# pl0q1n/RustyHGI

Hardware: AMD Instinct MI355X
Metric: Mpixels/s encode+decode, 4K grayscale level=4 Medium (higher is better)
Workload: dtype u8

## Files before the change

rustyhgi_amd/csrc/hgi_fused_impl.h:

```cpp
#include "hgi_dev.h"
#include "hgi_fastdiv.h"
#include "hgi_knobs.h"
#include "hgi_tilewalk.h"

namespace hgi {
namespace {

using namespace dev;

#ifndef HGI_TILE_H
#define HGI_TILE_H 64
#endif
#define HGI_LOG2(v) ((v) == 32 ? 5 : (v) == 16 ? 4 : (v) == 8 ? 3 : (v) == 4 ? 2 : 1)
#define HGI_CAT2(a, b) a##_##b
#define HGI_CAT(a, b) HGI_CAT2(a, b)
#define HGI_TILED(name) HGI_CAT(name, HGI_TILE_H)
#define HGI_LANE ((int)threadIdx.x)
constexpr int TW = kTileW;
constexpr int TH = HGI_TILE_H;
constexpr int MAXK = TH == 64 ? kFusedMaxLevels : TH == 32 ? kFusedMaxLevelsSmall : kFusedMaxLevelsTiny;
constexpr int NL = kThreads;
constexpr int CH = TW / 16;
constexpr int LCH = 3;
constexpr int HR = 6;
// ... 720 lines not shown
}

__device__ __forceinline__ void lattice_from_buf(const u8 *buf, u8 *rbuf, int nh)
{
    for (int i = HGI_LANE; i < (TH / 2 + nh) * CH; i += NL) {
        const int rr = i >> LCH, c = i & (CH - 1);
        *reinterpret_cast<v2u *>(rbuf + rr * S2 + 8 * c) = even_bytes(*reinterpret_cast<const v4u *>(buf + rr * S + 16 * c));
    }
    for (int i = HGI_LANE; i < HR * (TH / 2 + nh); i += NL) {
        const int hc = i / (TH / 2 + nh), rr = i - hc * (TH / 2 + nh);
        rbuf[RCOL + hc * HP2 + rr] = buf[HCOL + hc * HP + rr];
    }
}

__device__ __forceinline__ u32 gather_b0(v4u a)
{
    return __builtin_amdgcn_perm(a.y, a.x, 0x0c0c0400u) | __builtin_amdgcn_perm(a.w, a.z, 0x04000c0cu);
}

template <int INTERP, int EDGE = 0>
__device__ __forceinline__ void dec_level2_fast(u8 *buf, int rows = TH, int cols = TW)
{
    constexpr int N2 = (TH / 4) * CH;
#pragma unroll
    for (int it = 0; it < (N2 + NL - 1) / NL; ++it) {
        const bool on = N2 % NL == 0 || HGI_LANE + it * NL < N2;
        const int i = on ? HGI_LANE + it * NL : 0;
        u8 *r0 = buf + 2 * (i >> LCH) * S + 16 * (i & (CH - 1));
        v4u A = *reinterpret_cast<const v4u *>(r0);
        v4u B = *reinterpret_cast<const v4u *>(r0 + S);
        v4u C = *reinterpret_cast<const v4u *>(r0 + 2 * S);
        const int z0 = 2 * (i >> LCH);
        const bool last = (i & (CH - 1)) == CH - 1;
        u32 a16 = from_next_lane(A.x), c16 = from_next_lane(C.x);
        const u32 ha = buf[HCOL + z0], hc = buf[HCOL + z0 + 2];
        a16 = last ? ha : a16;
        c16 = last ? hc : c16;
        u32 ct = gather_b0(A), cb = gather_b0(C);
        u32 P = ct;
        if (INTERP == kInterpCrossed)
            P = pred4_crossed(ct, cb, __builtin_amdgcn_alignbyte(a16, ct, 1), __builtin_amdgcn_alignbyte(c16, cb, 1));
        u32 a0 = A.x, a1 = A.y, a2 = A.z, a3 = A.w, b0 = B.x, b1 = B.y, b2 = B.z, b3 = B.w;
        HGI_ADDB(a0, 2, P, 0); HGI_ADDB(a1, 2, P, 1); HGI_ADDB(a2, 2, P, 2); HGI_ADDB(a3, 2, P, 3);
        HGI_ADDB(b0, 0, P, 0); HGI_ADDB(b1, 0, P, 1); HGI_ADDB(b2, 0, P, 2); HGI_ADDB(b3, 0, P, 3);
        HGI_ADDB(b0, 2, P, 0); HGI_ADDB(b1, 2, P, 1); HGI_ADDB(b2, 2, P, 2); HGI_ADDB(b3, 2, P, 3);
        v4u An = {a0, a1, a2, a3}, Bn = {b0, b1, b2, b3};
        if (EDGE == 2 && cols < TW) {
            const v4u m = chunk_mask(cols - 16 * (i & (CH - 1)));
            An &= m;
            Bn &= m;
        }
        if (on && (!EDGE || 2 * z0 < rows)) *reinterpret_cast<v4u *>(r0) = An;
        if (on && (!EDGE || 2 * z0 + 2 < rows)) *reinterpret_cast<v4u *>(r0 + S) = Bn;
    }
}

template <int INTERP, int EDGE = 0>
__device__ __forceinline__ void dec_fine_fast(const u8 *buf, const Buf &b, const v4u (&odd)[NFINE], int rows = TH, int cols = TW)
{
    const int lane = HGI_LANE;
    const int rp0 = fine_pair0();
    const bool last = (lane & (CH - 1)) == CH - 1;
    const u8 *r0 = buf + rp0 * S + 16 * (lane & (CH - 1));
    const u8 *h0 = buf + HCOL + rp0;
    u32 voff = b.base + 2 * rp0 * b.W + 16 * (lane & (CH - 1));
#pragma unroll
    for (int it = 0; it < NFINE; ++it, r0 += (NL / CH) * S, h0 += NL / CH, voff += 2 * (NL / CH) * b.W) {
        v4u E = *reinterpret_cast<const v4u *>(r0);
        v4u O = odd[it];
        v4u F = *reinterpret_cast<const v4u *>(r0 + S);
        u32 e16 = from_next_lane(E.x), f16 = from_next_lane(F.x);
        const u32 he = h0[0], hf = h0[1];
        e16 = last ? he : e16;
        f16 = last ? hf : f16;
        uint2 c, fl;
        c.x = __builtin_amdgcn_perm(E.y, E.x, 0x06040200u);
        c.y = __builtin_amdgcn_perm(E.w, E.z, 0x06040200u);
        fl.x = __builtin_amdgcn_perm(F.y, F.x, 0x06040200u);
        fl.y = __builtin_amdgcn_perm(F.w, F.z, 0x06040200u);
        u32 P0, P1;
        pred8<INTERP>(c, e16, fl, f16, P0, P1);
        u32 e0 = E.x, e1 = E.y, e2 = E.z, e3 = E.w, o0 = O.x, o1 = O.y, o2 = O.z, o3 = O.w;
        HGI_ADDB(e0, 1, P0, 0); HGI_ADDB(e0, 3, P0, 1); HGI_ADDB(e1, 1, P0, 2); HGI_ADDB(e1, 3, P0, 3);
        HGI_ADDB(e2, 1, P1, 0); HGI_ADDB(e2, 3, P1, 1); HGI_ADDB(e3, 1, P1, 2); HGI_ADDB(e3, 3, P1, 3);
        HGI_ADDB(o0, 0, P0, 0); HGI_ADDB(o0, 1, P0, 0); HGI_ADDB(o0, 2, P0, 1); HGI_ADDB(o0, 3, P0, 1);
        HGI_ADDB(o1, 0, P0, 2); HGI_ADDB(o1, 1, P0, 2); HGI_ADDB(o1, 2, P0, 3); HGI_ADDB(o1, 3, P0, 3);
        HGI_ADDB(o2, 0, P1, 0); HGI_ADDB(o2, 1, P1, 0); HGI_ADDB(o2, 2, P1, 1); HGI_ADDB(o2, 3, P1, 1);
        HGI_ADDB(o3, 0, P1, 2); HGI_ADDB(o3, 1, P1, 2); HGI_ADDB(o3, 2, P1, 3); HGI_ADDB(o3, 3, P1, 3);
        v4u r0v = {e0, e1, e2, e3}, r1v = {o0, o1, o2, o3};
        if (EDGE == 2) {
            const int y = 2 * (rp0 + it * (NL / CH));
            store_rows_edge(r0v, r1v, b.rd, voff, __builtin_amdgcn_readfirstlane(b.W), cols - 16 * (lane & (CH - 1)), y < rows, y + 1 < rows);
        } else {
            store_row_pair(r0v, r1v, b.rd, voff, __builtin_amdgcn_readfirstlane(b.W));
        }
    }
}

template <int INTERP, bool IDENT, int EDGE = 0>
__device__ __forceinline__ void enc_level2_fast(u8 *buf, u8 *rbuf, const u8 *slut, Tile tl, u32 W, u32 H)
{
    const int rows = EDGE ? (int)(H - tl.Y0) : TH, cols = EDGE ? (int)(W - tl.X0) : TW;
    constexpr int N2 = (TH / 4) * CH, NIT = (N2 + NL - 1) / NL;
#pragma unroll
    for (int it = 0; it < NIT; ++it) {
        const bool on = N2 % NL == 0 || HGI_LANE + it * NL < N2;
        const int i = on ? HGI_LANE + it * NL : 0;
        const int g = i >> LCH, c = i & (CH - 1);
        u8 *r0 = buf + 2 * g * S + 16 * c;
        u8 *q0 = rbuf + 2 * g * S2 + 8 * c;
        const v4u A = *reinterpret_cast<const v4u *>(r0);
        const v4u B = *reinterpret_cast<const v4u *>(r0 + S);
        const v2u cu = *reinterpret_cast<const v2u *>(q0);
        const v2u cl = *reinterpret_cast<const v2u *>(q0 + 2 * S2);
        const u32 hu = rbuf[RCOL + 2 * g], hl = rbuf[RCOL + 2 * g + 2];
        LDS_ORDER();
        const bool last = c == CH - 1;
        u32 c8 = from_next_lane(cu.x), l8 = from_next_lane(cl.x);
        c8 = last ? hu : c8;
        l8 = last ? hl : l8;
        u32 ct = __builtin_amdgcn_perm(cu.y, cu.x, 0x06040200u), cb = __builtin_amdgcn_perm(cl.y, cl.x, 0x06040200u);
        u32 P = ct;
        if (INTERP == kInterpCrossed)
            P = pred4_crossed(ct, cb, __builtin_amdgcn_alignbyte(c8, ct, 1), __builtin_amdgcn_alignbyte(l8, cb, 1));
        u32 a0 = A.x, a1 = A.y, a2 = A.z, a3 = A.w, b0 = B.x, b1 = B.y, b2 = B.z, b3 = B.w;
        v2u n0, n1;
        if (IDENT) {
            const u32 pA = __builtin_amdgcn_perm(P, P, 0x0c010c00u), pB = __builtin_amdgcn_perm(P, P, 0x0c030c02u);
            n0.x = __builtin_amdgcn_perm(a0, ct, 0x0c010c00u) | __builtin_amdgcn_perm(a1, a0, 0x060c020cu);
            n0.y = __builtin_amdgcn_perm(a0, ct, 0x0c030c02u) | __builtin_amdgcn_perm(a3, a2, 0x060c020cu);
            n1.x = __builtin_amdgcn_perm(b1, b0, 0x06040200u);
            n1.y = __builtin_amdgcn_perm(b3, b2, 0x06040200u);
            const u32 m2 = 0x00FF0000u, m02 = 0x00FF00FFu;
            a0 = (a0 & ~m2) | (sub4(a0, pA << 16) & m2);
            a1 = (a1 & ~m2) | (sub4(a1, pA & m2) & m2);
            a2 = (a2 & ~m2) | (sub4(a2, pB << 16) & m2);
            a3 = (a3 & ~m2) | (sub4(a3, pB & m2) & m2);
            const u32 p0 = (pA & 0xFFu) * 0x00010001u, p1 = ((pA >> 16) & 0xFFu) * 0x00010001u;
            const u32 p2 = (pB & 0xFFu) * 0x00010001u, p3 = ((pB >> 16) & 0xFFu) * 0x00010001u;
            b0 = (b0 & ~m02) | (sub4(b0, p0) & m02);
            b1 = (b1 & ~m02) | (sub4(b1, p1) & m02);
            b2 = (b2 & ~m02) | (sub4(b2, p2) & m02);
            b3 = (b3 & ~m02) | (sub4(b3, p3) & m02);
        } else {
            const u32 NP = ~P;
            Q_PIX4(slut, P, NP, a0, 2, 0, a1, 2, 1, a2, 2, 2, a3, 2, 3);
            Q_PIX4(slut, P, NP, b0, 0, 0, b1, 0, 1, b2, 0, 2, b3, 0, 3);
            Q_PIX4(slut, P, NP, b0, 2, 0, b1, 2, 1, b2, 2, 2, b3, 2, 3);
            n0.x = __builtin_amdgcn_perm(ct, ct, 0x0c010c00u);
            n0.y = __builtin_amdgcn_perm(ct, ct, 0x0c030c02u);
            n1.x = 0;
            n1.y = 0;
            Q_REC(n0.x, 1, a0, 2, P, 0); Q_REC(n0.x, 3, a1, 2, P, 1); Q_REC(n0.y, 1, a2, 2, P, 2); Q_REC(n0.y, 3, a3, 2, P, 3);
            Q_REC(n1.x, 0, b0, 0, P, 0); Q_REC(n1.x, 1, b0, 2, P, 0); Q_REC(n1.x, 2, b1, 0, P, 1); Q_REC(n1.x, 3, b1, 2, P, 1);
            Q_REC(n1.y, 0, b2, 0, P, 2); Q_REC(n1.y, 1, b2, 2, P, 2); Q_REC(n1.y, 2, b3, 0, P, 3); Q_REC(n1.y, 3, b3, 2, P, 3);
        }
        v4u An = {a0, a1, a2, a3}, Bn = {b0, b1, b2, b3};
        if (EDGE == 2 && cols < TW) {
            const v4u m = chunk_mask(cols - 16 * c);
            const v2u m2 = chunk_mask2(cols - 16 * c);
            An &= m;
            Bn &= m;
            n0 &= m2;
            n1 &= m2;
        }
        if (on && (!EDGE || 4 * g < rows)) {
            *reinterpret_cast<v4u *>(r0) = An;
            *reinterpret_cast<v2u *>(q0) = n0;
        }
        if (on && (!EDGE || 4 * g + 2 < rows)) {
            *reinterpret_cast<v4u *>(r0 + S) = Bn;
            *reinterpret_cast<v2u *>(q0 + S2) = n1;
        }
        __builtin_amdgcn_sched_barrier(0);
    }
    LDS_ORDER();
    HGI_MARK("halo");
    enc_halo_pass<INTERP, IDENT>(buf, rbuf, slut, 2, tl, W, H);
}

template <int INTERP, bool IDENT, int EDGE = 0>
__device__ __forceinline__ void enc_fine_fast(const u8 *buf, const u8 *rbuf, const u8 *slut, const Buf &b,
                                              const v4u (&odd)[NFINE], int rows = TH, int cols = TW)
{
    const int lane = HGI_LANE;
    const int rp0 = fine_pair0();
    const bool last = (lane & (CH - 1)) == CH - 1;
    const u8 *r0 = buf + rp0 * S + 16 * (lane & (CH - 1));
    const u8 *c0 = rbuf + rp0 * S2 + 8 * (lane & (CH - 1));
    const u8 *h0 = rbuf + RCOL + rp0;
    u32 voff = b.base + 2 * rp0 * b.W + 16 * (lane & (CH - 1));
    const u32 Ws = __builtin_amdgcn_readfirstlane(b.W);
#ifndef HGI_FINE_BATCH
#define HGI_FINE_BATCH 2
#endif
    constexpr int NIT = NFINE, PAIR = NFINE >= HGI_FINE_BATCH ? HGI_FINE_BATCH : 1;
    static_assert(NIT % PAIR == 0, "fine level iterations come in pairs");
#pragma unroll
    for (int it = 0; it < NIT; it += PAIR) {
        v4u E_[PAIR], O_[PAIR];
        uint2 c_[PAIR], f_[PAIR];
        u32 hc_[PAIR], hf_[PAIR];
#pragma unroll
        for (int j = 0; j < PAIR; ++j) {
            const u8 *r = r0 + j * (NL / CH) * S, *c = c0 + j * (NL / CH) * S2, *h = h0 + j * (NL / CH);
            E_[j] = *reinterpret_cast<const v4u *>(r);
            O_[j] = odd[it + j];
            c_[j] = *reinterpret_cast<const uint2 *>(c);
            f_[j] = *reinterpret_cast<const uint2 *>(c + S2);
            hc_[j] = h[0];
            hf_[j] = h[1];
        }
#pragma unroll
        for (int j = 0; j < PAIR; ++j) {
            const v4u E = E_[j], O = O_[j];
            const uint2 c = c_[j], fl = f_[j];
            u32 c8 = from_next_lane(c.x), f8 = from_next_lane(fl.x);
            c8 = last ? hc_[j] : c8;
            f8 = last ? hf_[j] : f8;
            u32 P0, P1;
            pred8<INTERP>(c, c8, fl, f8, P0, P1);
            u32 e0 = E.x, e1 = E.y, e2 = E.z, e3 = E.w, g0 = O.x, g1 = O.y, g2 = O.z, g3 = O.w;
            if (IDENT) {
                const u32 odd = 0xFF00FF00u;
                const u32 pp0 = __builtin_amdgcn_perm(P0, P0, 0x01010000u), pp1 = __builtin_amdgcn_perm(P0, P0, 0x03030202u);
                const u32 pp2 = __builtin_amdgcn_perm(P1, P1, 0x01010000u), pp3 = __builtin_amdgcn_perm(P1, P1, 0x03030202u);
                e0 = sub4(e0, pp0 & odd); e1 = sub4(e1, pp1 & odd); e2 = sub4(e2, pp2 & odd); e3 = sub4(e3, pp3 & odd);
                g0 = sub4(g0, pp0); g1 = sub4(g1, pp1); g2 = sub4(g2, pp2); g3 = sub4(g3, pp3);
            } else {
                const u32 N0 = ~P0, N1 = ~P1;
                Q_PIX4(slut, P0, N0, e0, 1, 0, e0, 3, 1, e1, 1, 2, e1, 3, 3);
                Q_PIX4(slut, P1, N1, e2, 1, 0, e2, 3, 1, e3, 1, 2, e3, 3, 3);
                Q_PIX4(slut, P0, N0, g0, 0, 0, g0, 1, 0, g0, 2, 1, g0, 3, 1);
                Q_PIX4(slut, P0, N0, g1, 0, 2, g1, 1, 2, g1, 2, 3, g1, 3, 3);
                Q_PIX4(slut, P1, N1, g2, 0, 0, g2, 1, 0, g2, 2, 1, g2, 3, 1);
                Q_PIX4(slut, P1, N1, g3, 0, 2, g3, 1, 2, g3, 2, 3, g3, 3, 3);
            }
            v4u o0 = {e0, e1, e2, e3}, o1 = {g0, g1, g2, g3};
            const u32 vo = voff + j * 2 * (NL / CH) * Ws;
            if (EDGE == 2) {
                const int y = 2 * (rp0 + (it + j) * (NL / CH));
                store_rows_edge(o0, o1, b.rd, vo, Ws, cols - 16 * (lane & (CH - 1)), y < rows, y + 1 < rows);
            } else {
                store_row_pair(o0, o1, b.rd, vo, Ws);
            }
        }
        r0 += PAIR * (NL / CH) * S;
        c0 += PAIR * (NL / CH) * S2;
        h0 += PAIR * (NL / CH);
        voff += PAIR * 2 * (NL / CH) * Ws;
    }
}

__device__ __forceinline__ u8 *uniform_ptr(const u8 *p)
{
    const u64 a = reinterpret_cast<u64>(p);
    const u32 lo = __builtin_amdgcn_readfirstlane((u32)a), hi = __builtin_amdgcn_readfirstlane((u32)(a >> 32));
    return reinterpret_cast<u8 *>(((u64)hi << 32) | lo);
}

__device__ __forceinline__ Buf make_buf(const u8 *fr, u8 *out, u32 W, u32 H, Tile tl, u32 tail)
{
    Buf b;
    const u32 bytes = W * H;
    b.rs = __builtin_amdgcn_make_buffer_rsrc(uniform_ptr(fr), 0, bytes + tail, 0x00020000);
    b.rd = __builtin_amdgcn_make_buffer_rsrc(uniform_ptr(out), 0, bytes, 0x00020000);
    b.W = W;
    b.base = __builtin_amdgcn_readfirstlane(tl.Y0 * W + tl.X0);
    return b;
}

__device__ __forceinline__ Tile fast_tile(u32 t, const TileGrid &g)
{
    t = __builtin_amdgcn_readfirstlane(walk_position(t, g));
    const WalkTile w = walk_fast_tile(t, g);
    Tile tl;
    tl.frame = w.frame;
    tl.X0 = w.tx * TW;
    tl.Y0 = w.ty * TH;
    return tl;
}

__device__ __forceinline__ Tile edge_tile(u32 e, const TileGrid &g)
{
    const WalkTile w = walk_edge_tile(e, g);
    Tile tl;
    tl.frame = w.frame;
    tl.X0 = w.tx * TW;
    tl.Y0 = w.ty * TH;
    return tl;
}

struct TileCtx {
    Tile tl;
    Buf b;
};

#ifndef HGI_ARGS_EARLY
#define HGI_ARGS_EARLY 1
#endif
__device__ __forceinline__ void args_early(const u8 *src, const u8 *dst, const Frames &f, const TileGrid &g, u32 aligned, u32 k)
{
#if HGI_ARGS_EARLY
    asm volatile("" ::"s"(k), "s"(g.full_x), "s"(g.full_y), "s"(g.tiles_x), "s"(g.tiles_y));
    asm volatile("" ::"s"(src), "s"(dst), "s"(f.width), "s"(f.height), "s"(f.frame_stride), "s"(aligned), "s"(g.nedge), "s"(g.nf), "s"(g.xmode),
                 "s"(g.rr_own), "s"(g.rr_tail0), "s"(g.P), "s"(g.fd_P.m), "s"(g.fd_P.s1), "s"(g.fd_P.s2), "s"(g.reverse), "s"(g.tpf), "s"(g.fd_tpf.m),
                 "s"(g.fd_tpf.s1), "s"(g.fd_tpf.s2), "s"(g.nfull), "s"(g.rem_rows), "s"(g.band), "s"(g.ex), "s"(g.fd_band.m), "s"(g.fd_band.s1),
                 "s"(g.fd_band.s2), "s"(g.fd_rem.m), "s"(g.fd_rem.s1), "s"(g.fd_rem.s2));
#endif
}

__device__ __forceinline__ TileCtx fast_ctx(u32 t, const u8 *src, u8 *dst, const Frames &f, const TileGrid &g, u32 tail)
{
    TileCtx c;
    c.tl = fast_tile(t, g);
    c.b = make_buf(src + (size_t)c.tl.frame * f.frame_stride, dst + (size_t)c.tl.frame * f.frame_stride, f.width,
                   f.height, c.tl, tail);
    return c;
}

struct SeedRegs {
    u32 rec, q;
    int bx, by;
    bool on;
};

template <bool WANT_Q>
__device__ __forceinline__ SeedRegs seed_issue(const Seeds &sd, Tile tl, u32 k)
{
    const int ext = k >= 2 ? 2 : 1;
    const int nbx = (TW >> k) + ext, nby = (TH >> k) + ext;
    const int i = HGI_LANE;
    SeedRegs r;
    r.by = i / nbx;
    r.bx = i - r.by * nbx;
    r.on = i < nbx * nby;
    r.rec = r.q = 0;
    const u32 sx = (tl.X0 >> k) + r.bx, sy = (tl.Y0 >> k) + r.by;
    if (r.on && sx < sd.sw && sy < sd.sh) {
        const size_t at = (size_t)tl.frame * sd.stride + (size_t)sy * sd.sw + sx;
        r.rec = sd.rec[at];
        if (WANT_Q) r.q = sd.q[at];
    }
    return r;
}

__device__ __forceinline__ void dec_seed_commit(u8 *buf, const SeedRegs &r, u32 k)
{
    if (r.on) buf[laddr(r.bx << k, r.by << k)] = (u8)r.rec;
    LDS_ORDER();
}

constexpr int kConeMaxUp = 4;
__host__ __device__ constexpr int cone_n(int tile_px, int t)
{
    const int c = tile_px >> 4;
    int n = c + 2;
    for (int i = 0; i < t; ++i) n = (c % (2 << i) == 0 ? (n - 1) / 2 : n / 2) + 2;
    return n;
}
__host__ __device__ constexpr int cone_off(int t)
{
    int o = 0;
    for (int i = 1; i < t; ++i) o += cone_n(TW, i) * cone_n(TH, i);
    return o;
}
static_assert(cone_n(TW, 0) * cone_n(TH, 0) <= NL && cone_off(kConeMaxUp + 1) <= NL, "one lane per cone point");
static_assert(HR == 6 && cone_off(kConeMaxUp + 1) <= 2 * HP && cone_off(kConeMaxUp + 1) <= 2 * HP2, "the cone's arrays fit the two unused halo-column slots");
__device__ __forceinline__ u8 *cone_rec_array(u8 *buf) { return buf + HCOL + 4 * HP; }
__device__ __forceinline__ u8 *cone_q_array(u8 *rbuf) { return rbuf + RCOL + 4 * HP2; }
static_assert(cone_n(TW, 0) == 10 && cone_n(TW, 1) == 6 && cone_n(TW, 2) == 4 && cone_n(TW, 3) == 3 && cone_n(TW, 4) == 3, "cone widths of a 128-pixel tile");

struct ConeLane {
    u32 v, vq;
    u32 t;
    u32 src1;
    bool framed1;
    u32 from1, nx1;
    bool in1, down1;
    u32 src0, from0;
    bool on0, in0, down0;
};

__device__ __forceinline__ u32 cone_corner(u32 x, u32 y, u32 A, u32 B, u32 T, u32 nx2)
{
    const u32 m2 = (2u << T) - 1u;
    return (((y & ~m2) - (B & ~m2)) >> (T + 1)) * nx2 + (((x & ~m2) - (A & ~m2)) >> (T + 1));
}

struct FrameAt {
    __device__ __forceinline__ size_t operator()(size_t x, size_t y, u32 W) const { return y * W + x; }
};

template <bool WANT_Q, class At = FrameAt>
__device__ __forceinline__ ConeLane cone_issue(const u8 *__restrict__ fr, u32 W, u32 H, const Seeds &sd, Tile tl, At at = At{})
{
    const u32 up = sd.up, sw = ((W - 1u) >> 4) + 1u, sh = ((H - 1u) >> 4) + 1u;
    constexpr u32 o2 = cone_off(2), o3 = cone_off(3), o4 = cone_off(4), o5 = cone_off(5);
    constexpr u32 nx0 = cone_n(TW, 0), ny0 = cone_n(TH, 0);
    const u32 lane = HGI_LANE, A = tl.X0 >> 4, B = tl.Y0 >> 4;
    ConeLane c;
    const u32 t = 1u + (lane >= o2) + (lane >= o3) + (lane >= o4);
    const u32 first = t == 1 ? 0u : t == 2 ? o2 : t == 3 ? o3 : o4;
    const u32 nx = t == 1 ? (u32)cone_n(TW, 1) : t == 2 ? (u32)cone_n(TW, 2) : t == 3 ? (u32)cone_n(TW, 3) : (u32)cone_n(TW, 4);
    const u32 rcp = t == 1 ? 43u : t == 2 ? 64u : 86u;
    static_assert(cone_n(TW, 1) == 6 && cone_n(TW, 2) == 4 && cone_n(TW, 3) == 3 && cone_n(TW, 4) == 3, "reciprocals above");
    const u32 i = lane - first, iy = (i * rcp) >> 8, ix = i - iy * nx, m = (1u << t) - 1u;
    const u32 x = (A & ~m) + (ix << t), y = (B & ~m) + (iy << t);
    const bool on = lane < o5 && t <= up;
    c.t = on ? t : 0u;
    c.in1 = on && x < sw && y < sh;
    c.down1 = !((x | y) & (1u << t));
    c.nx1 = t == 1 ? (u32)cone_n(TW, 2) : (u32)cone_n(TW, 3);
    c.from1 = (t == 1 ? o2 : t == 2 ? o3 : o4) + cone_corner(x, y, A, B, t, c.nx1);
    const bool framed = x >= A && x < A + nx0 && y >= B && y < B + ny0;
    c.framed1 = c.in1 && framed;
    c.src1 = c.framed1 ? (u32)laddr((int)((x - A) << 4), (int)((y - B) << 4)) : 0u;
    c.v = c.vq = 0u;
    if (t == up && sd.rec) {
        c.framed1 = false;
        if (c.in1) {
            const size_t at = (size_t)tl.frame * sd.stride + (size_t)(y >> up) * sd.sw + (x >> up);
            c.v = sd.rec[at];
            if (WANT_Q) c.vq = sd.q[at];
        }
    } else if (c.in1 && !framed) {
        c.v = fr[at((size_t)x << 4, (size_t)y << 4, W)];
    }
    if (!WANT_Q || !sd.rec) c.vq = c.v;
    const u32 by = (lane * 26u) >> 8, bx = lane - by * nx0;
    static_assert(nx0 == 10, "reciprocal above");
    c.on0 = lane < nx0 * ny0;
    c.in0 = c.on0 && A + bx < sw && B + by < sh;
    c.down0 = !(((A + bx) | (B + by)) & 1u);
    c.from0 = cone_corner(A + bx, B + by, A, B, 0u, (u32)cone_n(TW, 1));
    c.src0 = c.on0 ? (u32)laddr((int)(bx << 4), (int)(by << 4)) : 0u;
    return c;
}

template <int INTERP, bool ENC, bool IDENT>
__device__ __forceinline__ void cone_code(u32 v, const u8 *r2, const u8 *q2, u32 nx2, bool down, bool inside, const u8 *slut, u32 &rec, u32 &q)
{
    const u32 c00 = r2[0], c01 = r2[nx2], c10 = r2[1], c11 = r2[nx2 + 1];
    const u32 q00 = ENC ? (u32)q2[0] : 0u;
    const u32 p = pred1<INTERP>(c00, c01, c10, c11);
    q = ENC ? quant1<IDENT>(v, p, slut) : v;
    rec = (p + q) & 255u;
    if (down) {
        rec = c00;
        q = q00;
    }
    if (!inside) rec = q = 0u;
}

template <int INTERP, bool ENC, bool IDENT>
__device__ __forceinline__ SeedRegs cone_finish(const ConeLane &c, u8 *buf, u8 *rbuf, u32 up, const u8 *slut)
{
    const u32 lane = HGI_LANE;
    u8 *R = cone_rec_array(buf), *Q = ENC ? cone_q_array(rbuf) : nullptr;
    const u32 v1 = c.framed1 ? (u32)buf[(int)c.src1] : c.v;
    const u32 v0 = c.on0 ? (u32)buf[(int)c.src0] : 0u;
    if (c.t == up) {
        R[lane] = (u8)v1;
        if (ENC) Q[lane] = (u8)(c.framed1 ? v1 : c.vq);
    }
    LDS_ORDER();
    for (u32 T = up - 1u; T >= 1u; --T) {
        if (c.t == T) {
            u32 rec, q;
            cone_code<INTERP, ENC, IDENT>(v1, R + c.from1, ENC ? Q + c.from1 : nullptr, c.nx1, c.down1, c.in1, slut, rec, q);
            R[lane] = (u8)rec;
            if (ENC) Q[lane] = (u8)q;
        }
        LDS_ORDER();
    }
    SeedRegs r;
    r.by = (int)((lane * 26u) >> 8);
    r.bx = (int)lane - r.by * cone_n(TW, 0);
    r.on = c.on0;
    r.rec = r.q = 0u;
    if (c.on0) cone_code<INTERP, ENC, IDENT>(v0, R + c.from0, ENC ? Q + c.from0 : nullptr, (u32)cone_n(TW, 1), c.down0, c.in0, slut, r.rec, r.q);
    LDS_ORDER();
    return r;
}

template <int INTERP>
__device__ __forceinline__ void dec_tile_fast(u8 *buf, const TileCtx &cur, const v4u (&odd)[NFINE], u32 k, u32 W, u32 H)
{
#define HGI_DEC_COARSE(SUB)                                                                    \
    if (k > HGI_LOG2(SUB)) {                                                                   \
        HGI_MARK("coarse");                                                                    \
        dec_cells<INTERP, false>(buf, SUB, cur.tl, W, H);                                      \
        HGI_MARK("halo");                                                                      \
        dec_halo_cells<INTERP>(buf, SUB, cur.tl, W, H);                                        \
        LDS_ORDER();                                                                           \
    }
    if (MAXK >= 6) HGI_DEC_COARSE(32)
    if (MAXK >= 5) HGI_DEC_COARSE(16)
    HGI_DEC_COARSE(8)
    HGI_DEC_COARSE(4)
#undef HGI_DEC_COARSE
    if (k >= 2) {
        HGI_MARK("level2");
        dec_level2_fast<INTERP>(buf);
        HGI_MARK("halo");
        dec_halo_cells<INTERP>(buf, 2, cur.tl, W, H);
        LDS_ORDER();
    }
    HGI_MARK("fine");
    dec_fine_fast<INTERP>(buf, cur.b, odd);
}

template <int INTERP, int EDGE>
__device__ __forceinline__ void dec_tile_edge(u8 *buf, const TileCtx &cur, const v4u (&odd)[NFINE], u32 k, u32 W, u32 H)
{
    const int rows = (int)(H - cur.tl.Y0), cols = (int)(W - cur.tl.X0);
#define HGI_DEC_EDGE_COARSE(SUB)                                   \
    if (k > HGI_LOG2(SUB)) {                                       \
        dec_cells<INTERP, true>(buf, SUB, cur.tl, W, H);           \
        dec_halo_cells<INTERP>(buf, SUB, cur.tl, W, H);            \
        LDS_ORDER();                                               \
    }
    if (MAXK >= 6) HGI_DEC_EDGE_COARSE(32)
    if (MAXK >= 5) HGI_DEC_EDGE_COARSE(16)
    HGI_DEC_EDGE_COARSE(8)
    HGI_DEC_EDGE_COARSE(4)
#undef HGI_DEC_EDGE_COARSE
    if (k >= 2) {
        dec_level2_fast<INTERP, EDGE>(buf, rows, cols);
        dec_halo_cells<INTERP>(buf, 2, cur.tl, W, H);
        LDS_ORDER();
    }
    dec_fine_fast<INTERP, EDGE>(buf, cur.b, odd, rows, cols);
}

__device__ __forceinline__ BlockRole block_role(const TileGrid &g) { return walk_block_role(blockIdx.x, g); }

#ifndef HGI_DEC_WAVES_PER_EU
#define HGI_DEC_WAVES_PER_EU 8
#endif
template <int INTERP, int SEEDED, int TILE_ROWS>
__global__ __launch_bounds__(NL) __attribute__((amdgpu_waves_per_eu(SEEDED == 2 ? HGI_DEC_WAVES_PER_EU - 2 : HGI_DEC_WAVES_PER_EU))) void k_dec_tiles(const u8 *__restrict__ src, u8 *__restrict__ dst, Frames f, u32 k,
                                                  Seeds sd, TileGrid g, u32 aligned)
{
    HGI_TL_ENTRY();
    args_early(src, dst, f, g, aligned, k);
    extern __shared__ __attribute__((aligned(16))) u8 smem[];
#ifdef HGI_ANALYZE_K
    k = HGI_ANALYZE_K;
#endif
    const int nh = k >= 2 ? (int)k : 1;
    u8 *buf = smem - HCOL;
    const u32 W = f.width, H = f.height;
#ifdef HGI_ANALYZE_K
    BlockRole role = block_role(g);
    role.edge = role.idle = false;
#else
    const BlockRole role = block_role(g);
#endif
    if (role.idle) return;
    if (!role.edge) {
        TileCtx cur = fast_ctx(role.index, src, dst, f, g, (aligned & 4u) ? 3u : 0u);
        Stage st;
        SeedRegs seeds;
        HGI_MARK("stage_issue");
        HGI_TL_START();
        ConeLane cone;
#if HGI_DEC_CONE_FIRST
        if (SEEDED == 2) cone = cone_issue<false>(src + (size_t)cur.tl.frame * f.frame_stride, W, H, sd, cur.tl);
#endif
        stage_issue<false>(st, cur.b, cur.tl, (int)k, nh);
        if (SEEDED == 1) seeds = seed_issue<false>(sd, cur.tl, k);
#if !HGI_DEC_CONE_FIRST
        if (SEEDED == 2) cone = cone_issue<false>(src + (size_t)cur.tl.frame * f.frame_stride, W, H, sd, cur.tl);
#endif
        HGI_MARK("stage_commit");
        stage_commit<false>(buf, nullptr, st, nh);
        LDS_ORDER();
        HGI_TL_STAGED();
        if (HGI_ODD_LATE) stage_issue_odd(st, cur.b);
        if (SEEDED == 2) seeds = cone_finish<INTERP, false, true>(cone, buf, nullptr, sd.up, nullptr);
        LDS_ORDER();
        if (SEEDED) dec_seed_commit(buf, seeds, k);
        dec_tile_fast<INTERP>(buf, cur, st.o, k, W, H);
        HGI_MARK("end");
        HGI_TL_END();
        return;
    }
    const Tile tl = edge_tile(role.index, g);
    const u8 *fr = src + (size_t)tl.frame * f.frame_stride;
    u8 *out = dst + (size_t)tl.frame * f.frame_stride;
    SeedRegs seeds;
    ConeLane cone;
    if (SEEDED == 1) seeds = seed_issue<false>(sd, tl, k);
    if (SEEDED == 2) cone = cone_issue<false>(fr, W, H, sd, tl);
    if (aligned & 2u) {
        TileCtx cur = {tl, make_buf(fr, out, W, H, tl, (aligned & 4u) ? 3u : 0u)};
        Stage st;
        stage_issue<true, true>(st, cur.b, tl, (int)k, nh);
        stage_commit<false>(buf, nullptr, st, nh);
        LDS_ORDER();
        if (SEEDED == 2) seeds = cone_finish<INTERP, false, true>(cone, buf, nullptr, sd.up, nullptr);
        if (SEEDED) dec_seed_commit(buf, seeds, k);
        if (tl.X0 + TW <= W && !(H & 1u))
            dec_tile_edge<INTERP, 1>(buf, cur, st.o, k, W, H);
        else
            dec_tile_edge<INTERP, 2>(buf, cur, st.o, k, W, H);
        return;
    }
    stage_tile_generic(buf, fr, W, H, tl, nh, (aligned & 1u) != 0);
    LDS_ORDER();
    if (SEEDED == 2) seeds = cone_finish<INTERP, false, true>(cone, buf, nullptr, sd.up, nullptr);
    if (SEEDED) dec_seed_commit(buf, seeds, k);
    for (int s = 1 << (k - 1); s >= 2; s >>= 1) {
        dec_cells<INTERP, true>(buf, s, tl, W, H);
        dec_halo_cells<INTERP>(buf, s, tl, W, H);
        LDS_ORDER();
    }
    dec_fine_generic<INTERP>(buf, fr, out, tl, W, H, (aligned & 1u) != 0);
}

template <int SEEDED>
__device__ __forceinline__ void enc_seed_commit(u8 *buf, u8 *rbuf, const SeedRegs &r, u32 k)
{
    if (SEEDED && r.on) {
        buf[laddr(r.bx << k, r.by << k)] = (u8)r.q;
        rbuf[laddr2(r.bx << k, r.by << k)] = (u8)r.rec;
    }
    LDS_ORDER();
}

template <int INTERP, bool IDENT, int EDGE>
__device__ __forceinline__ void enc_tile_edge(u8 *buf, u8 *rbuf, const u8 *slut, const TileCtx &cur,
                                              const v4u (&odd)[NFINE], u32 k, u32 W, u32 H)
{
#define HGI_ENC_EDGE_COARSE(SUB)                                                   \
    if (k > HGI_LOG2(SUB)) {                                                       \
        enc_cells<INTERP, IDENT, true>(buf, rbuf, slut, SUB, cur.tl, W, H);        \
        enc_halo_pass<INTERP, IDENT>(buf, rbuf, slut, SUB, cur.tl, W, H);          \
        LDS_ORDER();                                                               \
    }
    if (MAXK >= 6) HGI_ENC_EDGE_COARSE(32)
    if (MAXK >= 5) HGI_ENC_EDGE_COARSE(16)
    HGI_ENC_EDGE_COARSE(8)
    HGI_ENC_EDGE_COARSE(4)
#undef HGI_ENC_EDGE_COARSE
    if (k >= 2) {
        enc_level2_fast<INTERP, IDENT, EDGE>(buf, rbuf, slut, cur.tl, W, H);
        LDS_ORDER();
    }
    enc_fine_fast<INTERP, IDENT, EDGE>(buf, rbuf, slut, cur.b, odd, (int)(H - cur.tl.Y0), (int)(W - cur.tl.X0));
}

template <int INTERP, bool IDENT>
__device__ __forceinline__ void enc_tile_fast(u8 *buf, u8 *rbuf, const u8 *slut, const TileCtx &cur,
                                              const v4u (&odd)[NFINE], u32 k, u32 W, u32 H)
{
#define HGI_ENC_COARSE(SUB)                                                                    \
    if (k > HGI_LOG2(SUB)) {                                                                   \
        HGI_MARK("coarse");                                                                    \
        enc_level_coarse_fast<INTERP, IDENT>(buf, rbuf, slut, SUB, cur.tl, W, H);              \
        LDS_ORDER();                                                                           \
    }
    if (MAXK >= 6) HGI_ENC_COARSE(32)
    if (MAXK >= 5) HGI_ENC_COARSE(16)
    HGI_ENC_COARSE(8)
    HGI_ENC_COARSE(4)
#undef HGI_ENC_COARSE
    if (k >= 2) {
        HGI_MARK("level2");
        enc_level2_fast<INTERP, IDENT>(buf, rbuf, slut, cur.tl, W, H);
        LDS_ORDER();
    }
    HGI_MARK("fine");
    enc_fine_fast<INTERP, IDENT, 0>(buf, rbuf, slut, cur.b, odd);
}

#ifndef HGI_ENC_WAVES_PER_EU
#define HGI_ENC_WAVES_PER_EU 5
#endif
template <int INTERP, bool IDENT, int SEEDED, int TILE_ROWS>
__global__ __launch_bounds__(NL) __attribute__((amdgpu_waves_per_eu(IDENT ? HGI_ENC_WAVES_PER_EU - 1 : HGI_ENC_WAVES_PER_EU))) void k_enc_tiles(const u8 *__restrict__ src, u8 *__restrict__ dst, Frames f, u32 k,
                                                  Lut256 lut, Seeds sd, TileGrid g, u32 aligned)
{
    HGI_TL_ENTRY();
    args_early(src, dst, f, g, aligned, k);
    extern __shared__ __attribute__((aligned(16))) u8 smem[];
#ifdef HGI_ANALYZE_K
    k = HGI_ANALYZE_K;
#endif
    const int nh = k >= 2 ? (int)k : 1;
    u8 *slut = smem;
    u8 *buf = smem + 256 - HCOL;
    u8 *rbuf = smem + 256 + buf_bytes(nh) - RCOL;
    const u32 W = f.width, H = f.height;
#ifdef HGI_ANALYZE_K
    BlockRole role = block_role(g);
    role.edge = role.idle = false;
#else
    const BlockRole role = block_role(g);
#endif
    if (role.idle) return;
    u32 lutv = 0;
    if (!role.edge) {
        TileCtx cur = fast_ctx(role.index, src, dst, f, g, (aligned & 4u) ? 3u : 0u);
        Stage st;
        SeedRegs seeds;
        ConeLane cone;
        HGI_MARK("stage_issue");
        HGI_TL_START();
        stage_issue<false>(st, cur.b, cur.tl, (int)k, nh);
        if (SEEDED == 1) seeds = seed_issue<true>(sd, cur.tl, k);
        if (SEEDED == 2) cone = cone_issue<true>(src + (size_t)cur.tl.frame * f.frame_stride, W, H, sd, cur.tl);
        if (!IDENT) lutv = lut.w[HGI_LANE];
        HGI_MARK("stage_commit");
        stage_commit<true>(buf, rbuf, st, nh);
        if (!IDENT) reinterpret_cast<u32 *>(slut)[HGI_LANE] = lutv;
        LDS_ORDER();
        HGI_TL_STAGED();
        if (HGI_ODD_LATE) stage_issue_odd(st, cur.b);
        if (SEEDED == 2) seeds = cone_finish<INTERP, true, IDENT>(cone, buf, rbuf, sd.up, slut);
        enc_seed_commit<SEEDED>(buf, rbuf, seeds, k);
        enc_tile_fast<INTERP, IDENT>(buf, rbuf, slut, cur, st.o, k, W, H);
        HGI_MARK("end");
        HGI_TL_END();
        return;
    }
    const Tile tl = edge_tile(role.index, g);
    const u8 *fr = src + (size_t)tl.frame * f.frame_stride;
    u8 *out = dst + (size_t)tl.frame * f.frame_stride;
    SeedRegs seeds;
    if (SEEDED == 1) seeds = seed_issue<true>(sd, tl, k);
    ConeLane cone;
    if (SEEDED == 2) cone = cone_issue<true>(fr, W, H, sd, tl);
    if (aligned & 2u) {
        TileCtx cur = {tl, make_buf(fr, out, W, H, tl, (aligned & 4u) ? 3u : 0u)};
        Stage st;
        stage_issue<true, true>(st, cur.b, tl, (int)k, nh);
        if (!IDENT) lutv = lut.w[HGI_LANE];
        stage_commit<true>(buf, rbuf, st, nh);
        if (!IDENT) reinterpret_cast<u32 *>(slut)[HGI_LANE] = lutv;
        LDS_ORDER();
        if (SEEDED == 2) seeds = cone_finish<INTERP, true, IDENT>(cone, buf, rbuf, sd.up, slut);
        enc_seed_commit<SEEDED>(buf, rbuf, seeds, k);
        if (tl.X0 + TW <= W && !(H & 1u))
            enc_tile_edge<INTERP, IDENT, 1>(buf, rbuf, slut, cur, st.o, k, W, H);
        else
            enc_tile_edge<INTERP, IDENT, 2>(buf, rbuf, slut, cur, st.o, k, W, H);
        return;
    }
    if (!IDENT) reinterpret_cast<u32 *>(slut)[HGI_LANE] = lut.w[HGI_LANE];
    stage_tile_generic(buf, fr, W, H, tl, nh, (aligned & 1u) != 0);
    LDS_ORDER();
    lattice_from_buf(buf, rbuf, nh);
    LDS_ORDER();
    if (SEEDED == 2) seeds = cone_finish<INTERP, true, IDENT>(cone, buf, rbuf, sd.up, slut);
    enc_seed_commit<SEEDED>(buf, rbuf, seeds, k);
    for (int s = 1 << (k - 1); s >= 2; s >>= 1) {
        enc_cells<INTERP, IDENT, true>(buf, rbuf, slut, s, tl, W, H);
        enc_halo_pass<INTERP, IDENT>(buf, rbuf, slut, s, tl, W, H);
        LDS_ORDER();
    }
    enc_fine_generic<INTERP, IDENT>(buf, rbuf, slut, fr, out, tl, W, H, (aligned & 1u) != 0);
}

inline bool ptr16(const void *p) { return (reinterpret_cast<uintptr_t>(p) & 15u) == 0; }

struct FusedGeom {
    TileGrid g;
    u32 aligned;
    bool ok;
};

FusedGeom fused_geom(const void *a, const void *b, const Frames &f, u32 row_limit)
{
    FusedGeom r;
    TileGrid &g = r.g;
    g.tiles_x = (f.width + TW - 1) / TW;
    g.tiles_y = (f.height + TH - 1) / TH;
    if (row_limit && row_limit / TH < g.tiles_y) g.tiles_y = row_limit / TH;
    const bool aligned = f.width % 16 == 0 && f.frame_stride % 16 == 0 && ptr16(a) && ptr16(b);
    const bool fits32 = ((u64)f.height + 2 * TH + 64) * f.width + 1024 < (1ull << 32);
    const bool force_checked = HGI_SWITCH(HGI_FORCE_CHECKED);
    const uintptr_t end = reinterpret_cast<uintptr_t>(a) + (uintptr_t)(f.batch - 1) * f.frame_stride + (uintptr_t)f.width * f.height;
    const bool dword_rows = f.width % 4 == 0;
    const bool tail_ok = ((end - 1) >> 12) == ((end + 2) >> 12) && (f.batch == 1 || f.frame_stride >= (u64)f.width * f.height);
    const bool fast = fits32 && (dword_rows || tail_ok) && !force_checked;
    g.full_x = fast ? f.width / TW : 0;
    g.full_y = fast ? f.height / TH : 0;
    if (g.full_y > g.tiles_y) g.full_y = g.tiles_y;
    if (g.full_x == 0 || g.full_y == 0) g.full_x = g.full_y = 0;
    const u64 all = (u64)g.tiles_x * g.tiles_y * f.batch, nfast = (u64)g.full_x * g.full_y * f.batch;
    r.ok = all > 0 && all + 8 < (1ull << 31);
    g.nfast = (u32)nfast;
    g.nedge = (u32)(all - nfast);
    g.reverse = 0;
    g.band = HGI_TILE_BAND;
    g.xmode = 0;
    r.aligned = (aligned ? 1u : 0u) | (fast ? 2u : 0u) | (fast && !dword_rows ? 4u : 0u);
#ifdef HGI_TIMELINE
    g.timeline = g_timeline;
#endif
    return r;
}

inline u32 band_rows(const Frames &f, bool encode)
{
    const int forced = encode ? HGI_KNOB(HGI_ENC_BAND, 0) : HGI_KNOB(HGI_DEC_BAND, 0);
    if (forced > 0) return (u32)forced;
    const u64 cap = encode ? (4u << 20) : (2u << 20);
    u32 rows = HGI_TILE_BAND;
    while (rows > 1 && (u64)rows * TH * f.width > cap) rows >>= 1;
    return rows;
}


inline size_t lds_for_waves(size_t lds, int waves)
{
    if (waves <= 0) return lds;
    const size_t cap = ((size_t)160 * 1024 / (size_t)waves) & ~(size_t)255;
    return cap > lds ? cap : lds;
}

inline u32 xcd_mode(const TileGrid &g, bool encode)
{
    const int forced = HGI_KNOB(HGI_XCD_MODE, HGI_XCD_MODE);
    if (forced >= 0) return (u32)forced;
    return encode && (u64)g.nfast * TW * TH >= ((u64)HGI_XCD_EIGHTHS_FROM_GIB << 30) ? 0u : 1u;
}

}

#ifndef HGI_FUSED_NO_LAUNCHERS
#ifdef HGI_FUSED_DECODE
hipError_t HGI_TILED(launch_decode_fused)(const uint8_t *grid, uint8_t *img, const Frames &f, uint32_t k, int interp,
                                          const Seeds *seeds, hipStream_t s, uint32_t row_limit, int resident_tiles)
{
    FusedGeom r = fused_geom(grid, img, f, row_limit);
    if (!r.ok || k < 1 || k > (u32)MAXK) return hipErrorInvalidValue;
    r.g.reverse = HGI_KNOB(HGI_DEC_REVERSE, HGI_DEC_REVERSE_DEFAULT) ? 1u : 0u;
    r.g.band = band_rows(f, false);
    r.g.xmode = xcd_mode(r.g, false);
    finish_grid(r.g);
    const TileGrid &g = r.g;
    if (seeds && k < (uint32_t)kSeededMinLevels) return hipErrorInvalidValue;
    Seeds sd = seeds ? *seeds : Seeds{nullptr, nullptr, 0, 0, 0, 0};
    const bool cone = seeds && seeds->up != 0;
    if (cone && (k != 4 || sd.up > (u32)kConeMaxUp)) return hipErrorInvalidValue;
    if (seeds && !cone && !seeds->rec) return hipErrorInvalidValue;
    const dim3 b(NL);
    const int nh = k >= 2 ? (int)k : 1;
    const int dec_waves_forced = HGI_KNOB(HGI_DEC_WAVES, -1);
    const u64 tiles = (u64)g.nfast + g.nedge;
    int dec_waves = 0;
    if (resident_tiles >= 0)
        dec_waves = resident_tiles;
    else if (dec_waves_forced >= 0)
        dec_waves = dec_waves_forced;
    else if (tiles < 8192)
        dec_waves = 0;
    else if (!seeds)
        dec_waves = f.width > 4096 || k > 4 ? HGI_DEC_STREAM_WAVES_WIDE : k == 1 ? HGI_DEC_STREAM_WAVES_L1 : HGI_DEC_STREAM_WAVES;
    else
        dec_waves = tiles >= 65536 ? HGI_DEC_DEEP_WAVES : HGI_DEC_SHALLOW_WAVES;
    const size_t lds = lds_for_waves((size_t)buf_bytes(nh), dec_waves);
    const dim3 blocks(((g.nedge + 7u) & ~7u) + g.nfast);
#define HGI_DEC(I, SE) hipLaunchKernelGGL((k_dec_tiles<I, SE, TH>), blocks, b, lds, s, grid, img, f, k, sd, g, r.aligned)
#define HGI_DEC_I(I)                                                     \
    do {                                                                 \
        if (!seeds) HGI_DEC(I, 0);                                       \
        else if (cone) HGI_DEC(I, 2);                                    \
        else if constexpr (TH == 64) HGI_DEC(I, 1);                      \
        else return hipErrorInvalidValue;                                \
    } while (0)
    if (interp == kInterpCrossed) HGI_DEC_I(kInterpCrossed); else HGI_DEC_I(kInterpLeftTop);
#undef HGI_DEC_I
#undef HGI_DEC
    return hipGetLastError();
}

#endif

#ifdef HGI_FUSED_ENCODE
namespace {
hipError_t static_lds_is_empty(const void *kernel)
{
    hipFuncAttributes a;
    const hipError_t e = hipFuncGetAttributes(&a, kernel);
    if (e != hipSuccess) return e;
    return a.sharedSizeBytes == 0 ? hipSuccess : hipErrorInvalidDeviceFunction;
}
}

hipError_t HGI_TILED(launch_encode_fused)(const uint8_t *img, uint8_t *grid, const Frames &f, uint32_t k, int interp,
                                          const Lut256 &lut, bool ident, const Seeds *seeds, hipStream_t s, uint32_t row_limit)
{
    FusedGeom r = fused_geom(img, grid, f, row_limit);
    if (!r.ok || k < 1 || k > (u32)MAXK) return hipErrorInvalidValue;
    r.g.band = band_rows(f, true);
    r.g.xmode = xcd_mode(r.g, true);
    finish_grid(r.g);
    const TileGrid &g = r.g;
    if (seeds && k < (uint32_t)kSeededMinLevels) return hipErrorInvalidValue;
    Seeds sd = seeds ? *seeds : Seeds{nullptr, nullptr, 0, 0, 0, 0};
    const bool cone = seeds && seeds->up != 0;
    if (cone && (k != 4 || sd.up > (u32)kConeMaxUp)) return hipErrorInvalidValue;
    if (seeds && (!seeds->rec != !seeds->q || (!cone && !seeds->rec))) return hipErrorInvalidValue;
    const dim3 b(NL);
    const int nh = k >= 2 ? (int)k : 1;
    const int enc_waves = HGI_KNOB(HGI_ENC_WAVES, 0);
    const size_t lds = lds_for_waves((size_t)buf_bytes(nh) + ((rbuf_bytes(nh) + 15) & ~15) + 256, enc_waves);
    const dim3 blocks(((g.nedge + 7u) & ~7u) + g.nfast);
#define HGI_ENC(I, ID, SE)                                                                                        \
    do {                                                                                                          \
        static const hipError_t lds0 = static_lds_is_empty(reinterpret_cast<const void *>(&k_enc_tiles<I, ID, SE, TH>)); \
        if (lds0 != hipSuccess) return lds0;                                                                      \
        hipLaunchKernelGGL((k_enc_tiles<I, ID, SE, TH>), blocks, b, lds, s, img, grid, f, k, lut, sd, g, r.aligned); \
    } while (0)
#define HGI_ENC_ID(I, ID)                                                     \
    do {                                                                      \
        if (cone) HGI_ENC(I, ID, 2);                                          \
        else if (!seeds) HGI_ENC(I, ID, 0);                                   \
        else if constexpr (TH == 64) HGI_ENC(I, ID, 1);                       \
        else return hipErrorInvalidValue;                                     \
    } while (0)
#define HGI_ENC_I(I)                                                          \
    do {                                                                      \
        if (ident) HGI_ENC_ID(I, true); else HGI_ENC_ID(I, false);            \
    } while (0)
    if (interp == kInterpCrossed) HGI_ENC_I(kInterpCrossed); else HGI_ENC_I(kInterpLeftTop);
#undef HGI_ENC_I
#undef HGI_ENC_ID
#undef HGI_ENC
    return hipGetLastError();
}

#endif
#endif

}
```

rustyhgi_amd/csrc/hgi_tilewalk.h:

```cpp
#pragma once
#include <stdint.h>

#include "hgi_fastdiv.h"

#if defined(__HIPCC__)
#define HGI_WALK_FN __host__ __device__ __forceinline__
#else
#define HGI_WALK_FN inline
#endif
#ifndef HGI_TILE_ORDER
#define HGI_TILE_ORDER 0
#endif

namespace hgi {
namespace {

struct TileGrid {
    uint32_t tiles_x, tiles_y;
    uint32_t full_x, full_y;
    uint32_t nfast, nedge;
    uint32_t reverse;
    uint32_t band;
    uint32_t xmode;
    uint32_t ex, nf;
    uint32_t tpf, P, nfull, rem_rows;
    uint32_t rr_own, rr_tail0;
    FastDiv fd_tpf, fd_P, fd_band, fd_rem, fd_ex;
#ifdef HGI_TIMELINE
    uint64_t *timeline;
#endif
};

struct WalkTile {
    uint32_t frame, tx, ty;
};

HGI_WALK_FN uint32_t range_first(uint32_t ntiles, uint32_t x) { return x * (ntiles >> 3) + (x < (ntiles & 7u) ? x : (ntiles & 7u)); }

HGI_WALK_FN uint32_t walk_position(uint32_t t, const TileGrid &g) { return g.reverse ? g.nf - 1u - t : t; }

HGI_WALK_FN WalkTile walk_fast_tile(uint32_t t, const TileGrid &g)
{
    WalkTile tl;
    tl.frame = fdiv(t, g.fd_tpf);
    const uint32_t tt = t - tl.frame * g.tpf;
    uint32_t ty, tx;
#if HGI_TILE_ORDER == 0
    ty = fdiv(tt, g.fd_ex);
    tx = tt - ty * g.ex;
#else
    {
        uint32_t rows, row0, r;
        if (tt < g.nfull) {
            const uint32_t band = fdiv(tt, g.fd_P);
            r = tt - band * g.P;
            row0 = band * g.band;
            rows = g.band;
            tx = fdiv(r, g.fd_band);
        } else {
            rows = g.rem_rows;
            r = tt - g.nfull;
            row0 = g.full_y - rows;
            tx = fdiv(r, g.fd_rem);
        }
        ty = row0 + (r - tx * rows);
    }
#endif
    tl.tx = tx;
    tl.ty = ty;
    return tl;
}

HGI_WALK_FN WalkTile walk_edge_tile(uint32_t e, const TileGrid &g)
{
    const uint32_t right = (g.tiles_x - g.full_x) * g.tiles_y;
    const uint32_t epf = right + g.full_x * (g.tiles_y - g.full_y);
    WalkTile tl;
    tl.frame = e / epf;
    uint32_t i = e - tl.frame * epf, tx, ty;
    if (i < right) {
        const uint32_t w = g.tiles_x - g.full_x;
        ty = i / w;
        tx = g.full_x + (i - ty * w);
    } else {
        i -= right;
        ty = g.full_y + i / g.full_x;
        tx = i % g.full_x;
    }
    tl.tx = tx;
    tl.ty = ty;
    return tl;
}

struct BlockRole {
    bool edge, idle;
    uint32_t index;
};

HGI_WALK_FN BlockRole walk_block_role(uint32_t b, const TileGrid &g)
{
    const uint32_t ne8 = (g.nedge + 7u) & ~7u;
    BlockRole r;
    r.edge = b < ne8;
    r.idle = r.edge && b >= g.nedge;
    const uint32_t fb = b - ne8;
    r.index = r.edge ? b : range_first(g.nf, fb & 7u) + (fb >> 3);
    if (!r.edge && g.xmode == 1) {
        const uint32_t x = fb & 7u, sq = fb >> 3;
        if (sq < g.rr_own) {
            const uint32_t round = fdiv(sq, g.fd_P);
            r.index = (round * 8u + x) * g.P + (sq - round * g.P);
        } else {
            r.index = g.rr_tail0 + range_first(g.nf - g.rr_tail0, x) + (sq - g.rr_own);
        }
    }
    return r;
}

inline void finish_grid(TileGrid &g)
{
    g.ex = g.full_x;
    g.nf = g.nfast;
    if (g.band < 1) g.band = 1;
    g.tpf = g.ex * g.full_y;
    g.P = g.band * g.ex;
    g.nfull = (g.full_y / g.band) * g.P;
    g.rem_rows = g.full_y % g.band;
    g.fd_tpf = make_fastdiv(g.tpf);
    g.fd_P = make_fastdiv(g.P);
    g.fd_band = make_fastdiv(g.band);
    g.fd_rem = make_fastdiv(g.rem_rows);
    g.fd_ex = make_fastdiv(g.ex);
    g.rr_own = g.rr_tail0 = 0;
    if (g.xmode != 1 || g.rem_rows != 0 || g.P == 0 || g.nf == 0) {
        g.xmode = 0;
    } else {
        const uint32_t nb8 = (g.nf / g.P) & ~7u;
        g.rr_own = (nb8 >> 3) * g.P;
        g.rr_tail0 = nb8 * g.P;
    }
}

}
}
```

Before: 1.609 million.

## Add XCD round-robin mode that handles partial row bands by reordering tiles

Adds a new XCD scheduling mode (2) for cases where the tile rows do not divide evenly into bands. Previously these cases fell back to plain contiguous ranges. The tile walk is reordered so that all full bands of every frame come first, followed by all remainder bands, which lets the full bands be dealt round-robin across the eight XCDs in whole bands. This is meant to improve L2 locality per XCD on decode and small encodes. In exchange, the tile-index decode gains a branch and an extra fast-division.

New measurement: 1.603 million. Within noise of the previous version (-0.4%).

```diff
diff --git a/rustyhgi_amd/csrc/hgi_fused_impl.h b/rustyhgi_amd/csrc/hgi_fused_impl.h
--- a/rustyhgi_amd/csrc/hgi_fused_impl.h
+++ b/rustyhgi_amd/csrc/hgi_fused_impl.h
@@ -1046,10 +1046,10 @@
 __device__ __forceinline__ void args_early(const u8 *src, const u8 *dst, const Frames &f, const TileGrid &g, u32 aligned, u32 k)
 {
 #if HGI_ARGS_EARLY
-    asm volatile("" ::"s"(k), "s"(g.full_x), "s"(g.full_y), "s"(g.tiles_x), "s"(g.tiles_y));
+    asm volatile("" ::"s"(k), "s"(g.full_x), "s"(g.full_y), "s"(g.tiles_x), "s"(g.tiles_y), "s"(g.a_tiles));
     asm volatile("" ::"s"(src), "s"(dst), "s"(f.width), "s"(f.height), "s"(f.frame_stride), "s"(aligned), "s"(g.nedge), "s"(g.nf), "s"(g.xmode),
-                 "s"(g.rr_own), "s"(g.rr_tail0), "s"(g.P), "s"(g.fd_P.m), "s"(g.fd_P.s1), "s"(g.fd_P.s2), "s"(g.reverse), "s"(g.tpf), "s"(g.fd_tpf.m),
-                 "s"(g.fd_tpf.s1), "s"(g.fd_tpf.s2), "s"(g.nfull), "s"(g.rem_rows), "s"(g.band), "s"(g.ex), "s"(g.fd_band.m), "s"(g.fd_band.s1),
+                 "s"(g.rr_own), "s"(g.rr_tail0), "s"(g.P), "s"(g.fd_P.m), "s"(g.fd_P.s1), "s"(g.fd_P.s2), "s"(g.reverse), "s"(g.ftpf), "s"(g.fd_ftpf.m),
+                 "s"(g.fd_ftpf.s1), "s"(g.fd_ftpf.s2), "s"(g.nfull), "s"(g.rem_rows), "s"(g.band), "s"(g.ex), "s"(g.fd_band.m), "s"(g.fd_band.s1),
                  "s"(g.fd_band.s2), "s"(g.fd_rem.m), "s"(g.fd_rem.s1), "s"(g.fd_rem.s2));
 #endif
 }
@@ -1570,7 +1570,7 @@
 {
     const int forced = HGI_KNOB(HGI_XCD_MODE, HGI_XCD_MODE);
     if (forced >= 0) return (u32)forced;
-    return encode && (u64)g.nfast * TW * TH >= ((u64)HGI_XCD_EIGHTHS_FROM_GIB << 30) ? 0u : 1u;
+    return encode && (u64)g.nfast * TW * TH >= ((u64)HGI_XCD_EIGHTHS_FROM_GIB << 30) ? 0u : 2u;
 }
 
 }
diff --git a/rustyhgi_amd/csrc/hgi_tilewalk.h b/rustyhgi_amd/csrc/hgi_tilewalk.h
--- a/rustyhgi_amd/csrc/hgi_tilewalk.h
+++ b/rustyhgi_amd/csrc/hgi_tilewalk.h
@@ -25,7 +25,10 @@
     uint32_t ex, nf;
     uint32_t tpf, P, nfull, rem_rows;
     uint32_t rr_own, rr_tail0;
+    uint32_t a_tiles, ftpf;
+    uint32_t rem_P;
     FastDiv fd_tpf, fd_P, fd_band, fd_rem, fd_ex;
+    FastDiv fd_ftpf, fd_remP;
 #ifdef HGI_TIMELINE
     uint64_t *timeline;
 #endif
@@ -42,8 +45,15 @@
 HGI_WALK_FN WalkTile walk_fast_tile(uint32_t t, const TileGrid &g)
 {
     WalkTile tl;
-    tl.frame = fdiv(t, g.fd_tpf);
-    const uint32_t tt = t - tl.frame * g.tpf;
+    uint32_t tt;
+    if (t < g.a_tiles) {
+        tl.frame = fdiv(t, g.fd_ftpf);
+        tt = t - tl.frame * g.ftpf;
+    } else {
+        const uint32_t u = t - g.a_tiles;
+        tl.frame = fdiv(u, g.fd_remP);
+        tt = g.nfull + (u - tl.frame * g.rem_P);
+    }
     uint32_t ty, tx;
 #if HGI_TILE_ORDER == 0
     ty = fdiv(tt, g.fd_ex);
@@ -105,7 +115,7 @@
     r.idle = r.edge && b >= g.nedge;
     const uint32_t fb = b - ne8;
     r.index = r.edge ? b : range_first(g.nf, fb & 7u) + (fb >> 3);
-    if (!r.edge && g.xmode == 1) {
+    if (!r.edge && g.xmode != 0) {
         const uint32_t x = fb & 7u, sq = fb >> 3;
         if (sq < g.rr_own) {
             const uint32_t round = fdiv(sq, g.fd_P);
@@ -132,13 +142,20 @@
     g.fd_rem = make_fastdiv(g.rem_rows);
     g.fd_ex = make_fastdiv(g.ex);
     g.rr_own = g.rr_tail0 = 0;
-    if (g.xmode != 1 || g.rem_rows != 0 || g.P == 0 || g.nf == 0) {
+    g.rem_P = g.rem_rows * g.ex;
+    const uint32_t whole = g.tpf ? (g.nf / g.tpf) * g.nfull : 0;
+    if (g.xmode == 2) g.xmode = g.rem_rows == 0 ? 1u : whole == 0 ? 0u : 2u;
+    if ((g.xmode == 1 && g.rem_rows != 0) || g.xmode > 2 || g.P == 0 || g.nf == 0) {
         g.xmode = 0;
-    } else {
-        const uint32_t nb8 = (g.nf / g.P) & ~7u;
+    } else if (g.xmode != 0) {
+        const uint32_t nb8 = ((g.xmode == 2 ? whole : g.nf) / g.P) & ~7u;
         g.rr_own = (nb8 >> 3) * g.P;
         g.rr_tail0 = nb8 * g.P;
     }
+    g.a_tiles = g.xmode == 2 ? whole : g.nf;
+    g.ftpf = g.xmode == 2 ? g.nfull : g.tpf;
+    g.fd_ftpf = make_fastdiv(g.ftpf);
+    g.fd_remP = make_fastdiv(g.rem_P);
 }
 
 }
```
